# PARC-projects/video-query-algorithms

Measured on AMD Instinct MI355X. Metric: clips/sec TSN feature-extract, higher is better.
Workload: dtype f32; 1 GPU; configs[1]: TSN BN-Inception RGB, 224x224x3, T=3, B=32/GPU (96 crops/step), crops in HBM; global_batch=32, parallelism=dp1

## Files before the change

video-query-algorithms_amd/csrc/vq_tsn.hip:

```cpp
#include <algorithm>
#include <cmath>
#include <cstring>
#include <map>
#include <set>
#include <tuple>
#include <type_traits>
#include <vector>

#include "vq_common.h"
#include "vq_tsn_kernels.h"
#include "host/vq_block_pool.h"

using namespace vq;

typedef float floatx16 __attribute__((ext_vector_type(16)));
typedef float floatx4 __attribute__((ext_vector_type(4)));
typedef unsigned uintx4 __attribute__((__vector_size__(4 * sizeof(unsigned))));

__global__ void preprocess_kernel(const uint8_t* __restrict__ src, float* __restrict__ dst, int64_t nchunk, int C, int Cpad,
                                  const float* __restrict__ mean) {
    const int64_t i = (int64_t)blockIdx.x * blockDim.x + threadIdx.x;
    if (i >= nchunk) return;
    const int cpp = Cpad >> 2;
    const int64_t p = i / cpp;
// ... 294 lines not shown
    floatx16 acc[TM][TN];
#pragma unroll
    for (int i = 0; i < TM; ++i)
#pragma unroll
        for (int j = 0; j < TN; ++j)
#pragma unroll
            for (int r = 0; r < 16; ++r) acc[i][j][r] = 0.f;

    floatx4 bias_v[TN];
    ConvSeg seg_v[TN];
#pragma unroll
    for (int j = 0; j < TN; ++j) {
        const int nb_ = n0 + wn * (BN / WN) + 32 * j;
        const int n = nb_ + (lane & 7) * 4;
        bias_v[j] = *reinterpret_cast<const floatx4*>(a.bias + (n < a.Cout ? n : 0));
        seg_v[j] = a.segs[ks * a.seg_stride + (nb_ < a.Cout ? nb_ >> 5 : 0)];
    }

    const int nk = (a.ksplit > 1 ? a.k_per : a.Kp) / BK;
    VQ_LOAD_TILES(0)
    VQ_STORE_TILES(0)
    __syncthreads();
    for (int kc = 0; kc < nk; ++kc) {
        const int buf = kc & 1;
        if (kc + 1 < nk) VQ_LOAD_TILES(kc + 1)
#pragma unroll
        for (int kk = 0; kk < BK / 8; ++kk) {
            floatx4 af[TM], bf[TN];
#pragma unroll
            for (int i = 0; i < TM; ++i) af[i] = *reinterpret_cast<const floatx4*>(&sm.a[buf][arow0 + 32 * i][kk * 8 + half * 4]);
#pragma unroll
            for (int j = 0; j < TN; ++j) bf[j] = *reinterpret_cast<const floatx4*>(&sm.b[buf][brow0 + 32 * j][kk * 8 + half * 4]);
#pragma unroll
            for (int s = 0; s < 4; ++s)
#pragma unroll
                for (int i = 0; i < TM; ++i)
#pragma unroll
                    for (int j = 0; j < TN; ++j)
                        acc[i][j] = __builtin_amdgcn_mfma_f32_32x32x2f32(af[i][s], bf[j][s], acc[i][j], 0, 0, 0);
        }
        if (kc + 1 < nk) VQ_STORE_TILES(buf ^ 1)
        __syncthreads();
    }

    VQ_EPILOGUE()
#undef VQ_LOAD_TILES
#undef VQ_STORE_TILES
}

#ifndef VQ_PIPE_WPE
#define VQ_PIPE_WPE 4
#endif
template <int BM, int BN, int WM, int WN, int BK, bool SMALL_CIN>
__global__ __launch_bounds__(256) __attribute__((amdgpu_waves_per_eu(BM * BN == 128 * 64 && BK == 16 ? VQ_PIPE_WPE : 1, 8)))
void conv_igemm_pipe_kernel(ConvArgs a) {
    static_assert(WM * WN == 4, "4 waves per workgroup");
    constexpr int NT = 256;
    constexpr int TM = BM / WM / 32, TN = BN / WN / 32;
    constexpr int CPR = BK / 4;
    constexpr int NA = (BM * CPR + NT - 1) / NT, NB = (BN * CPR + NT - 1) / NT;
    constexpr int NKK = BK / 8;
    constexpr int MFK = 4 * TM * TN;
    constexpr int NMF = NKK * MFK;
    constexpr int NFR = TM + TN;
    constexpr int NG = NA + NB;
    constexpr int NFREE = NMF - (NKK - 1) * NFR;
    static_assert(NFREE >= 2 * NG, "not enough MFMA gaps for the staging slices");
    constexpr bool EARLY = (NKK - 1) * (MFK - NFR) >= NG && NFREE - NFR >= 2 * NG;
    extern __shared__ __attribute__((aligned(16))) char smem_raw[];
    ConvSmem<BM, BN, BK>& sm = *reinterpret_cast<ConvSmem<BM, BN, BK>*>(smem_raw);

    const int tid = threadIdx.x;
    const int n_tiles = a.tiles_m * a.tiles_n;
    const int ks = a.ksplit > 1 ? (int)blockIdx.x / n_tiles : 0;
    const int kbeg = ks * a.k_per;
    const int tile = xcd_remap(blockIdx.x - ks * n_tiles, n_tiles);
    const int tm = (int)magic_div((unsigned)tile, a.m_tiles_n);
    const int m0 = tm * BM;
    const int n0 = (tile - tm * a.tiles_n) * BN;
    const unsigned img0 = full_div((unsigned)m0, a.d_howo), rem0 = (unsigned)m0 - img0 * (unsigned)(a.Ho * a.Wo);
    const unsigned oh0 = full_div(rem0, a.d_wo), ow0 = rem0 - oh0 * (unsigned)a.Wo;

    const __amdgpu_buffer_rsrc_t in_rsrc = __builtin_amdgcn_make_buffer_rsrc(const_cast<float*>(a.in), 0, a.in_bytes, 0x00020000);
    const __amdgpu_buffer_rsrc_t w_rsrc = __builtin_amdgcn_make_buffer_rsrc(const_cast<float*>(a.w), 0, a.w_bytes, 0x00020000);
    int a_off[NA];
    unsigned long long a_mask[NA];
    int a_row[NA], a_col[NA];
    const unsigned HW = (unsigned)(a.H * a.W);
#pragma unroll
    for (int i = 0; i < NA; ++i) {
        const int c = tid + NT * i;
        a_row[i] = c / CPR;
        a_col[i] = c % CPR;
        const bool ok = m0 + a_row[i] < a.M && a_row[i] < BM;
        const unsigned lin = ow0 + (unsigned)a_row[i];
        const unsigned q1 = umul24(lin, a.s_wo) >> kRecipShift;
        const unsigned ly = oh0 + q1;
        const unsigned q2 = umul24(ly, a.s_ho) >> kRecipShift;
        const int ow = (int)(lin - umul24(q1, (unsigned)a.Wo)), oh = (int)(ly - umul24(q2, (unsigned)a.Ho));
        const int ih0 = imul24(oh, a.stride) - a.pad, iw0 = imul24(ow, a.stride) - a.pad;
        a_off[i] = (imul24((int)umul24(img0 + q2, HW) + imul24(ih0, a.W) + iw0, a.Cs_in) + a.coff_in + (SMALL_CIN ? 0 : imul24(a_col[i], a.col_off))) * 4;
        unsigned long long mask = 0;
        for (int th = 0; th < a.k; ++th)
            for (int tw = 0; tw < a.kw; ++tw)
                if (ok && (unsigned)(ih0 + th) < (unsigned)a.H && (unsigned)(iw0 + tw) < (unsigned)a.W) mask |= 1ull << (th * a.kw + tw);
        a_mask[i] = mask;
    }
    unsigned b_off[NB];
    int b_row[NB], b_col[NB];
#pragma unroll
    for (int i = 0; i < NB; ++i) {
        const int c = tid + NT * i;
        b_row[i] = c / CPR;
        b_col[i] = c % CPR;
        const int n = n0 + b_row[i];
        b_off[i] = (n < a.Cout && b_row[i] < BN) ? (unsigned)((imul24(n, a.Kp) + b_col[i] * 4 + kbeg) * 4) : 0xFFFFFFFFu;
    }

    floatx4 ra[2][NA], rb[2][NB];
    int kh = 0, kw = 0, c0 = 0, tap = 0;
    unsigned a_voff[NA];
    if (!SMALL_CIN && kbeg > 0) {
        tap = kbeg / a.Cin;
        c0 = kbeg - tap * a.Cin;
        kh = tap / a.kw;
        kw = tap - kh * a.kw;
    }
    {
        const int tap_pix0 = ((kh * a.W + kw) * a.Cs_in) * 4;
#pragma unroll
        for (int i = 0; i < NA; ++i) a_voff[i] = ((a_mask[i] >> tap) & 1ull) ? (unsigned)(a_off[i] + tap_pix0) : 0xFFFFFFFFu;
    }
    const int c_step = a.c_step ? a.c_step : BK;
    const unsigned cpt = (unsigned)a.Cin >> 2, inv_cpt = 65536u / cpt + 1u, inv_k = 65536u / (unsigned)a.kw + 1u;

    const int wave = __builtin_amdgcn_readfirstlane(tid >> 6), lane = tid & 63, l31 = lane & 31, half = lane >> 5;
    const int wm = wave / WN, wn = wave % WN;
    const int arow0 = wm * (BM / WM) + l31, brow0 = wn * (BN / WN) + l31;
    floatx16 acc[TM][TN];
#pragma unroll
    for (int i = 0; i < TM; ++i)
#pragma unroll
        for (int j = 0; j < TN; ++j)
#pragma unroll
            for (int r = 0; r < 16; ++r) acc[i][j][r] = 0.f;
    floatx4 bias_v[TN];
    ConvSeg seg_v[TN];
#pragma unroll
    for (int j = 0; j < TN; ++j) {
        const int nb_ = n0 + wn * (BN / WN) + 32 * j;
        const int n = nb_ + (lane & 7) * 4;
        bias_v[j] = *reinterpret_cast<const floatx4*>(a.bias + (n < a.Cout ? n : 0));
        seg_v[j] = a.segs[ks * a.seg_stride + (nb_ < a.Cout ? nb_ >> 5 : 0)];
    }

#define VQ_G_LOAD(IDX, KC, SET)                                                                                \
    {                                                                                                          \
        if ((IDX) < NA) {                                                                                      \
            const int ii = (IDX) < NA ? (IDX) : 0;                                                             \
            unsigned off;                                                                                      \
            if (SMALL_CIN) {                                                                                   \
                const unsigned g_ = (unsigned)(KC) * CPR + a_col[ii];                                          \
                const unsigned tap_ = (g_ * inv_cpt) >> 16, c4_ = g_ - tap_ * cpt;                             \
                const unsigned th_ = (tap_ * inv_k) >> 16, tw_ = tap_ - th_ * a.kw;                            \
                const unsigned ok_ = (unsigned)(a_mask[ii] >> (tap_ & 63u)) & (tap_ < 64u ? 1u : 0u);          \
                off = ok_ ? (unsigned)(a_off[ii] + (int)(((th_ * a.W + tw_) * a.Cs_in + c4_ * 4) * 4)) : 0xFFFFFFFFu; \
            } else {                                                                                           \
                off = a_voff[ii];                                                                              \
            }                                                                                                  \
            ra[SET][ii] = __builtin_bit_cast(floatx4, __builtin_amdgcn_raw_buffer_load_b128(in_rsrc, off, SMALL_CIN ? 0 : c0 * 4, 0)); \
        } else {                                                                                               \
            const int ii = (IDX) >= NA ? (IDX) - NA : 0;                                                       \
            rb[SET][ii] = __builtin_bit_cast(floatx4, __builtin_amdgcn_raw_buffer_load_b128(w_rsrc, b_off[ii], (KC) * (BK * 4), 0)); \
        }                                                                                                      \
    }
#define VQ_G_STORE(IDX, BUF, SET)                                                                              \
    {                                                                                                          \
        if ((IDX) < NA) {                                                                                      \
            const int ii = (IDX) < NA ? (IDX) : 0;                                                             \
            if ((BM * CPR) % NT == 0 || a_row[ii] < BM)                                                        \
                *reinterpret_cast<floatx4*>(&sm.a[BUF][a_row[ii]][a_col[ii] * 4]) = ra[SET][ii];               \
        } else {                                                                                               \
            const int ii = (IDX) >= NA ? (IDX) - NA : 0;                                                       \
            if ((BN * CPR) % NT == 0 || b_row[ii] < BN)                                                        \
                *reinterpret_cast<floatx4*>(&sm.b[BUF][b_row[ii]][b_col[ii] * 4]) = rb[SET][ii];               \
        }                                                                                                      \
    }
#define VQ_ADVANCE_TAP()                                                                     \
    if (!SMALL_CIN) {                                                                        \
        c0 += c_step;                                                                        \
        if (c0 >= a.Cin) {                                                                   \
            c0 = 0;                                                                          \
            ++tap;                                                                           \
            if (++kw == a.kw) {                                                              \
                kw = 0;                                                                      \
                ++kh;                                                                        \
            }                                                                                \
            asm volatile("" ::: "memory");                  \
            const int tap_pix = ((kh * a.W + kw) * a.Cs_in) * 4;                             \
            _Pragma("unroll") for (int i = 0; i < NA; ++i)                                   \
                a_voff[i] = ((a_mask[i] >> tap) & 1ull) ? (unsigned)(a_off[i] + tap_pix) : 0xFFFFFFFFu; \
        }                                                                                    \
    }
#define VQ_PIPE_STEP(BUF, KC, DO_STORE, DO_LOAD, SS, SL)                                                       \
    {                                                                                                          \
        if (!EARLY) {                                                                                          \
            _Pragma("unroll") for (int i = 0; i < TM; ++i)                                                     \
                fa[0][i] = *reinterpret_cast<const floatx4*>(&sm.a[BUF][arow0 + 32 * i][half * 4]);            \
            _Pragma("unroll") for (int j = 0; j < TN; ++j)                                                     \
                fb[0][j] = *reinterpret_cast<const floatx4*>(&sm.b[BUF][brow0 + 32 * j][half * 4]);            \
        }                                                                                                      \
        _Pragma("unroll") for (int q = 0; q < NMF; ++q) {                                                      \
            const int kk = q / MFK, r = q % MFK, s_ = r / (TM * TN), i_ = (r / TN) % TM, j_ = r % TN;          \
            acc[i_][j_] = __builtin_amdgcn_mfma_f32_32x32x2f32(fa[kk & 1][i_][s_], fb[kk & 1][j_][s_], acc[i_][j_], 0, 0, 0); \
            if (kk + 1 < NKK && r < NFR) {                                                                     \
                if (r < TM)                                                                                    \
                    fa[(kk + 1) & 1][r < TM ? r : 0] = *reinterpret_cast<const floatx4*>(                      \
                        &sm.a[BUF][arow0 + 32 * (r < TM ? r : 0)][(kk + 1) * 8 + half * 4]);                   \
                else                                                                                           \
                    fb[(kk + 1) & 1][r >= TM ? r - TM : 0] = *reinterpret_cast<const floatx4*>(                \
                        &sm.b[BUF][brow0 + 32 * (r >= TM ? r - TM : 0)][(kk + 1) * 8 + half * 4]);             \
            } else if (EARLY && (DO_STORE) && kk + 1 == NKK && r < NFR) {                                      \
                if (r < TM)                                                                                    \
                    fa[0][r < TM ? r : 0] = *reinterpret_cast<const floatx4*>(                                 \
                        &sm.a[(BUF) ^ 1][arow0 + 32 * (r < TM ? r : 0)][half * 4]);                            \
                else                                                                                           \
                    fb[0][r >= TM ? r - TM : 0] = *reinterpret_cast<const floatx4*>(                           \
                        &sm.b[(BUF) ^ 1][brow0 + 32 * (r >= TM ? r - TM : 0)][half * 4]);                      \
            } else {                                                                                           \
                const int fidx = q - (kk + 1 < NKK ? (kk + 1) * NFR : (NKK - 1) * NFR + (EARLY && (DO_STORE) ? NFR : 0)); \
                if ((DO_STORE) && fidx < NG) {                                                                 \
                    VQ_G_STORE(fidx < NG ? fidx : 0, (BUF) ^ 1, SS)                                            \
                    if (EARLY && fidx == NG - 1) __syncthreads();            \
                } else if ((DO_LOAD) && fidx >= NG && fidx < 2 * NG)                                           \
                    VQ_G_LOAD(fidx - NG < NG ? fidx - NG : 0, (KC) + 2, SL)                                    \
            }                                                                                                  \
            __builtin_amdgcn_sched_barrier(0);                                                                 \
        }                                                                                                      \
    }

    const int nk = (a.ksplit > 1 ? a.k_per : a.Kp) / BK;
    _Pragma("unroll") for (int i = 0; i < NG; ++i) VQ_G_LOAD(i, 0, 0)
    _Pragma("unroll") for (int i = 0; i < NG; ++i) VQ_G_STORE(i, 0, 0)
    if (nk > 1) {
        VQ_ADVANCE_TAP()
        _Pragma("unroll") for (int i = 0; i < NG; ++i) VQ_G_LOAD(i, 1, 1)
    }
    __syncthreads();
    floatx4 fa[2][TM], fb[2][TN];
    if (EARLY) {
#pragma unroll
        for (int i = 0; i < TM; ++i) fa[0][i] = *reinterpret_cast<const floatx4*>(&sm.a[0][arow0 + 32 * i][half * 4]);
#pragma unroll
        for (int j = 0; j < TN; ++j) fb[0][j] = *reinterpret_cast<const floatx4*>(&sm.b[0][brow0 + 32 * j][half * 4]);
    }
#define VQ_END_BARRIER()                                                     \
    {                                                                        \
        if (EARLY) {                                                         \
            asm volatile("s_waitcnt lgkmcnt(%0)" ::"n"(NFR) : "memory");     \
            __builtin_amdgcn_s_barrier();                                    \
            asm volatile("" ::: "memory");                                   \
        } else {                                                             \
            __syncthreads();                                                 \
        }                                                                    \
    }
    const int n_steady = nk > 2 ? nk - 2 : 0;
    int kc = 0;
    for (; kc + 1 < n_steady; kc += 2) {
        VQ_ADVANCE_TAP()
        VQ_PIPE_STEP(0, kc, true, true, 1, 0)
        VQ_END_BARRIER()
        VQ_ADVANCE_TAP()
        VQ_PIPE_STEP(1, kc + 1, true, true, 0, 1)
        VQ_END_BARRIER()
    }
    if (kc < n_steady) {
        VQ_ADVANCE_TAP()
        VQ_PIPE_STEP(0, kc, true, true, 1, 0)
        VQ_END_BARRIER()
        ++kc;
    }
    if (kc + 1 < nk) {
        if (kc & 1) {
            VQ_PIPE_STEP(1, kc, true, false, 0, 0)
        } else {
            VQ_PIPE_STEP(0, kc, true, false, 1, 1)
        }
        VQ_END_BARRIER()
        ++kc;
    }
    if (kc & 1) {
        VQ_PIPE_STEP(1, kc, false, false, 0, 0)
    } else {
        VQ_PIPE_STEP(0, kc, false, false, 0, 0)
    }
    VQ_EPILOGUE_BUF()
#undef VQ_G_LOAD
#undef VQ_G_STORE
#undef VQ_ADVANCE_TAP
#undef VQ_PIPE_STEP
#undef VQ_END_BARRIER
}

template <int BM, int BN, int WM, int WN>
__global__ __launch_bounds__(256) void pool_gemm_kernel(ConvArgs a) {
    static_assert(WM * WN == 4, "4 waves per workgroup");
    static_assert(BM == 64 || BM == 128, "two staged chunks per thread and slab");
    constexpr int TM = BM / WM / 32, TN = BN / WN / 32;
    constexpr int SLAB = 2048 / BM;
    constexpr int CPS = SLAB / 4;
    constexpr int GS = SLAB / 8;
    extern __shared__ __attribute__((aligned(16))) char smem_raw[];
    float* As = reinterpret_cast<float*>(smem_raw);
    const int K = a.Cin, pitch = K + 4;
    const int tid = threadIdx.x;
    const int tile = xcd_remap(blockIdx.x, a.tiles_m * a.tiles_n);
    const int m0 = (tile / a.tiles_n) * BM, n0 = (tile % a.tiles_n) * BN;
    const __amdgpu_buffer_rsrc_t in_rsrc = __builtin_amdgcn_make_buffer_rsrc(const_cast<float*>(a.in), 0, a.in_bytes, 0x00020000);
    const __amdgpu_buffer_rsrc_t w_rsrc = __builtin_amdgcn_make_buffer_rsrc(const_cast<float*>(a.w), 0, a.w_bytes, 0x00020000);

    const int wave = tid >> 6, lane = tid & 63, l31 = lane & 31, half = lane >> 5;
    const int wm = wave / WN, wn = wave % WN;
    floatx4 bias_v[TN];
    ConvSeg seg_v[TN];
    unsigned b_voff[TN];
#pragma unroll
    for (int j = 0; j < TN; ++j) {
        const int nb_ = n0 + wn * (BN / WN) + 32 * j;
        const int n = nb_ + (lane & 7) * 4;
        bias_v[j] = *reinterpret_cast<const floatx4*>(a.bias + (n < a.Cout ? n : 0));
        seg_v[j] = a.segs[nb_ < a.Cout ? nb_ >> 5 : 0];
        b_voff[j] = nb_ + l31 < a.Cout ? (unsigned)(((nb_ + l31) * a.Kp + half * 4) * 4) : 0xFFFFFFFFu;
    }

    unsigned tap_base[2], tap_ok[2];
    int a_dst[2];
    const int px = a.Cs_in * 4, rowb = a.W * px;
    {
        const int HoWo = a.Ho * a.Wo;
#pragma unroll
        for (int u = 0; u < 2; ++u) {
            const int idx = tid + 256 * u, row = idx / CPS, col = idx % CPS;
            const int m = m0 + row;
            const bool ok = m < a.M;
            const int mm = ok ? m : 0;
            const int n_img = mm / HoWo, rem = mm - n_img * HoWo;
            const int oh = rem / a.Wo, ow = rem - oh * a.Wo;
            const int ih0 = oh * a.pool_s, iw0 = ow * a.pool_s;
            tap_base[u] = ok ? (unsigned)((((n_img * a.H + ih0) * a.W + iw0) * a.Cs_in + a.coff_in + col * 4) * 4) : 0xFFFFFFFFu;
            const int nvy = min(3, a.H - ih0), nvx = min(3, a.W - iw0);
            unsigned mask = 0;
#pragma unroll
            for (int t = 0; t < 9; ++t)
                if (ok && t / 3 < nvy && t % 3 < nvx) mask |= 1u << t;
            tap_ok[u] = mask;
            a_dst[u] = row * pitch + col * 4;
        }
    }
    floatx4 v[2][9];
#define VQ_PG_TAPS(S)                                                                                               \
    _Pragma("unroll") for (int u = 0; u < 2; ++u) {                                                                 \
        unsigned inside = tap_ok[u];                                                                                \
        asm volatile("" : "+v"(inside));  \
        _Pragma("unroll") for (int t = 0; t < 9; ++t)                                                               \
            v[u][t] = __builtin_bit_cast(floatx4, __builtin_amdgcn_raw_buffer_load_b128(                            \
                in_rsrc, tap_base[u] + (((inside >> t) & 1u) ? (unsigned)((t / 3) * rowb + (t % 3) * px) : 0u), (S) * (SLAB * 4), 0)); \
    }
#define VQ_PG_POOL(S)                                                                                               \
    _Pragma("unroll") for (int u = 0; u < 2; ++u) {                                                                 \
        floatx4 r;                                                                                                  \
        _Pragma("unroll") for (int e = 0; e < 4; ++e) {                                                             \
            const float x = __builtin_fmaxf(__builtin_fmaxf(v[u][0][e], v[u][1][e]), v[u][2][e]);                  \
            const float y = __builtin_fmaxf(__builtin_fmaxf(v[u][3][e], v[u][4][e]), v[u][5][e]);                  \
            const float z = __builtin_fmaxf(__builtin_fmaxf(v[u][6][e], v[u][7][e]), v[u][8][e]);                  \
            r[e] = __builtin_fmaxf(__builtin_fmaxf(x, y), z);                                                       \
        }                                                                                                           \
        *reinterpret_cast<floatx4*>(As + a_dst[u] + (S) * SLAB) = r;                                                \
    }

    floatx16 acc[TM][TN];
#pragma unroll
    for (int i = 0; i < TM; ++i)
#pragma unroll
        for (int j = 0; j < TN; ++j)
#pragma unroll
            for (int r = 0; r < 16; ++r) acc[i][j][r] = 0.f;
    const float* a_frag = As + (wm * (BM / WM) + l31) * pitch + half * 4;
    floatx4 fa[2][TM], fbs[2][GS][TN];
#define VQ_PG_FETCH_B(SET, S)                                                                                       \
    _Pragma("unroll") for (int q = 0; q < GS; ++q)                                                                  \
        _Pragma("unroll") for (int j = 0; j < TN; ++j)                                                              \
            fbs[SET][q][j] = __builtin_bit_cast(floatx4, __builtin_amdgcn_raw_buffer_load_b128(w_rsrc, b_voff[j], ((S) * GS + q) * 32, 0));
#define VQ_PG_FETCH_A(SET, G)                                                                                       \
    _Pragma("unroll") for (int i = 0; i < TM; ++i)                                                                  \
        fa[SET][i] = *reinterpret_cast<const floatx4*>(a_frag + 32 * i * pitch + (G) * 8);
#define VQ_PG_MFMA(SET, BSET, Q)                                                                                    \
    _Pragma("unroll") for (int s_ = 0; s_ < 4; ++s_)                                                                \
        _Pragma("unroll") for (int i = 0; i < TM; ++i)                                                              \
            _Pragma("unroll") for (int j = 0; j < TN; ++j)                                                          \
                acc[i][j] = __builtin_amdgcn_mfma_f32_32x32x2f32(fa[SET][i][s_], fbs[BSET][Q][j][s_], acc[i][j], 0, 0, 0);
#define VQ_PG_SLAB(S, BSET)                                                                                         \
    {                                                                                                               \
        const bool more = (S) + 1 < ns;                                                                             \
        if (more) {                                                                                                 \
            VQ_PG_FETCH_B((BSET) ^ 1, (S) + 1)                                                                      \
            VQ_PG_TAPS((S) + 1)                                              \
        }                                                                                                           \
        VQ_PG_FETCH_A(0, (S) * GS)                                                                                  \
        __builtin_amdgcn_sched_barrier(0);                                                                          \
        _Pragma("unroll") for (int q = 0; q < GS; ++q) {                                                            \
            if (q + 1 < GS) VQ_PG_FETCH_A((q + 1) & 1, (S) * GS + q + 1)                                            \
            __builtin_amdgcn_sched_barrier(0);                                                                      \
            VQ_PG_MFMA(q & 1, BSET, q)                                                                              \
            __builtin_amdgcn_sched_barrier(0);                                                                      \
        }                                                                                                           \
        if (more) {                                                                                                 \
            VQ_PG_POOL((S) + 1)                                                                                     \
            __syncthreads();                                  \
        }                                                                                                           \
    }

    const int ns = K / SLAB;
    VQ_PG_FETCH_B(0, 0)
    VQ_PG_TAPS(0)
    VQ_PG_POOL(0)
    __syncthreads();
    int s = 0;
    for (; s + 1 < ns; s += 2) {
        VQ_PG_SLAB(s, 0)
        VQ_PG_SLAB(s + 1, 1)
    }
    if (s < ns) VQ_PG_SLAB(s, 0)
#undef VQ_PG_SLAB
#undef VQ_PG_TAPS
#undef VQ_PG_POOL
#undef VQ_PG_FETCH_A
#undef VQ_PG_FETCH_B
#undef VQ_PG_MFMA
    VQ_EPILOGUE()
}

template <bool IS_MAX>
__global__ __launch_bounds__(256) void pool_kernel(PoolArgs a) {
    const int64_t i = (int64_t)blockIdx.x * blockDim.x + threadIdx.x;
    if (i < a.total) pool_one<IS_MAX>(a, i);
}

__global__ void gavgpool_kernel(const float* __restrict__ in, float* __restrict__ out, int n, int HW, int Cs_in, int coff_in,
                                int C, int Cs_out, int coff_out) {
    const int i = blockIdx.x * blockDim.x + threadIdx.x;
    if (i >= n * C) return;
    const int c = i % C, img = i / C;
    const float* p = in + (size_t)img * HW * Cs_in + coff_in + c;
    float acc = 0.f;
    for (int q = 0; q < HW; ++q) acc += p[(size_t)q * Cs_in];
    out[(size_t)img * Cs_out + coff_out + c] = acc / (float)HW;
}

__global__ void splitk_combine_kernel(const float* __restrict__ part, int ksplit, size_t slice_stride, int M, int Cout,
                                      const float* __restrict__ bias, int relu, float* __restrict__ out, int Cs_out) {
    const int64_t i = (int64_t)blockIdx.x * blockDim.x + threadIdx.x;
    const int c4 = Cout / 4;
    if (i >= (int64_t)M * c4) return;
    const int m = (int)(i / c4), n = (int)(i - (int64_t)m * c4) * 4;
    floatx4 v = *reinterpret_cast<const floatx4*>(part + (size_t)m * Cout + n);
    for (int q = 1; q < ksplit; ++q) v += *reinterpret_cast<const floatx4*>(part + q * slice_stride + (size_t)m * Cout + n);
    v += *reinterpret_cast<const floatx4*>(bias + n);
    if (relu) {
        v[0] = fmaxf(v[0], 0.f);
        v[1] = fmaxf(v[1], 0.f);
        v[2] = fmaxf(v[2], 0.f);
        v[3] = fmaxf(v[3], 0.f);
    }
    *reinterpret_cast<floatx4*>(out + (size_t)m * Cs_out + n) = v;
}

constexpr int kMaxFusedT = 16;
__global__ void gavgpool_consensus_kernel(const float* __restrict__ in, float* __restrict__ out, double* __restrict__ feat, int T,
                                          int HW, int Cs_in, int coff_in, int C, int Cs_out, int coff_out) {
    __shared__ float pooled[kMaxFusedT][64];
    const int c = blockIdx.x * 64 + threadIdx.x, t = threadIdx.y, b = blockIdx.y;
    float v = 0.f;
    if (c < C) {
        const int img = b * T + t;
        const float* p = in + (size_t)img * HW * Cs_in + coff_in + c;
        float acc = 0.f;
        int q = 0;
        for (; q + 7 <= HW; q += 7) {
            float x[7];
#pragma unroll
            for (int u = 0; u < 7; ++u) x[u] = p[(size_t)(q + u) * Cs_in];
#pragma unroll
            for (int u = 0; u < 7; ++u) acc += x[u];
        }
        for (; q < HW; ++q) acc += p[(size_t)q * Cs_in];
        v = acc / (float)HW;
        out[(size_t)img * Cs_out + coff_out + c] = v;
    }
    pooled[t][threadIdx.x] = v;
    __syncthreads();
    if (t == 0 && c < C) {
        double cons = (double)pooled[0][threadIdx.x];
        for (int s = 1; s < T; ++s) cons = cons + (double)pooled[s][threadIdx.x];
        feat[(size_t)b * C + c] = cons / (double)T;
    }
}

__global__ void consensus_kernel(const float* __restrict__ per_snippet, double* __restrict__ feat, int B, int T, int D, int Cs) {
    const int i = blockIdx.x * blockDim.x + threadIdx.x;
    if (i >= B * D) return;
    const int d = i % D, b = i / D;
    double acc = (double)per_snippet[(size_t)(b * T) * Cs + d];
    for (int t = 1; t < T; ++t) acc = acc + (double)per_snippet[(size_t)(b * T + t) * Cs + d];
    feat[i] = acc / (double)T;
}

static inline double first_layer_k2c(const vq_input_desc& in, const vq_layer_desc& L) {
    if (L.src != 0) return (double)L.k * L.k * L.cin;
    const int k = (in.s2d_pad >= 0 && in.s2d_kernel > 0) ? in.s2d_kernel : L.k;
    return (double)k * k * in.c;
}

static inline bool is_wino(int op) { return op == VQ_OP_CONV_WINOGRAD || op == VQ_OP_CONV_WINOGRAD16; }
static inline bool is_conv(int op) { return op == VQ_OP_CONV || is_wino(op); }

struct LaunchItem {
    int kind = 0;
    std::vector<int> layers;
    int max_crops = 0;
};

struct vq_tsn {
    std::mutex mu;
    int device = 0;
    hipStream_t stream = nullptr;
    int cus = 256;
    int max_crops = 0;
    int in_channels = 0;
    vq_input_desc input = {0, 0, 0, -1, 0};
    std::vector<vq_tensor_desc> tensors;
    std::vector<vq_layer_desc> layers;
    std::vector<LaunchItem> items;
    std::vector<int> item_of_layer;
    int consensus_layer = -1;
    std::map<int, std::vector<int>> tuned;
    std::map<int, int> split_pref;
    std::set<int> tuned_borrowed;
    bool autotune = true;
    bool group_wino = true;
    bool group_pool = true;
    bool poison = false;
    int forced_tile = -1;
    std::vector<float*> slots;
    std::vector<size_t> slot_bytes;
    size_t blob_bytes = 0;
    float* zeros = nullptr;
    ConvSeg* seg_table = nullptr;
    std::vector<int> seg_table_off;
    std::vector<int> ksplit;
    float* split_scratch = nullptr;
    size_t split_slice_floats = 0;
    size_t split_crop_floats = 0;
    float* zero_bias = nullptr;
    float* blob = nullptr;
    int64_t blob_floats = 0;
    int feature_slot = -1, D = 0;
    uint8_t* crops_dev = nullptr;
    size_t crops_cap = 0;
    float* mean_dev = nullptr;
    std::vector<float> mean_cached;
    double* feat_dev = nullptr;
    double flops_per_crop = 0;
    int last_crops = 0;
    int cur_T = 1;
    bool fused_consensus = false;
    int profile_depth = 0;
    int profile_count = 0;
    int profile_every = 1;
    int profile_tick = 0;
    bool profile_split = false;
    std::vector<hipEvent_t> events;
    int crop_off = 0;
    int n_split = 1;
    std::vector<int> split_parts;
    hipStream_t ls = nullptr;
    hipEvent_t ev_start = nullptr, ev_stop = nullptr;
    std::vector<hipStream_t> split_streams;
    hipEvent_t fork_ev = nullptr;
    std::vector<hipEvent_t> join_ev;
};

static vq::BlockPool& device_pool() {
    static vq::BlockPool p(vq::BlockPool::cap_from_env());
    return p;
}
void vq::device_pool_trim() {
    for (void* blk : device_pool().drain()) (void)hipFree(blk);
}
static hipError_t pool_alloc(int device, size_t bytes, void** out) {
    if (void* blk = device_pool().take(device, bytes)) {
        *out = blk;
        return hipSuccess;
    }
    hipError_t e = hipMalloc(out, bytes);
    if (e == hipErrorOutOfMemory) {
        (void)hipGetLastError();
        vq::device_pool_trim();
        e = hipMalloc(out, bytes);
    }
    return e;
}
static void pool_free(int device, void* p, size_t bytes) {
    if (!p) return;
    if (!device_pool().give(device, p, bytes)) (void)hipFree(p);
}

static void tsn_free(vq_tsn* net) {
    for (hipEvent_t e : net->events) (void)hipEventDestroy(e);
    net->events.clear();
    for (hipEvent_t e : net->join_ev)
        if (e) (void)hipEventDestroy(e);
    if (net->fork_ev) (void)hipEventDestroy(net->fork_ev);
    for (hipStream_t st : net->split_streams)
        if (st) (void)hipStreamDestroy(st);
    for (size_t i = 0; i < net->slots.size(); ++i) pool_free(net->device, net->slots[i], i < net->slot_bytes.size() ? net->slot_bytes[i] : 0);
    pool_free(net->device, net->blob, net->blob_bytes);
    if (net->zeros) (void)hipFree(net->zeros);
    if (net->seg_table) (void)hipFree(net->seg_table);
    pool_free(net->device, net->split_scratch, net->split_slice_floats * 4 * sizeof(float));
    if (net->zero_bias) (void)hipFree(net->zero_bias);
    if (net->crops_dev) (void)hipFree(net->crops_dev);
    if (net->mean_dev) (void)hipFree(net->mean_dev);
    if (net->feat_dev) (void)hipFree(net->feat_dev);
}

enum : int { kConv = 1, kPipe = 2, kPool = 4, kGemm = 8 };

constexpr size_t kPoolGemmMaxLds = 64 * 1024;
static size_t pool_gemm_lds(int bm, int K) { return std::max((size_t)bm * (K + 4) * sizeof(float), (size_t)4 * 32 * 36 * sizeof(float)); }

static bool pixel_walk_ok(const ConvArgs& a) {
    const long long n_img = cdiv(a.M, a.Ho * a.Wo);
    return n_img * a.H * a.W < (1 << 23) && a.Cs_in < (1 << 23) && a.Kp < (1 << 23) && a.Cout < (1 << 23) && a.stride < (1 << 23) &&
           recip22_ok((unsigned)a.Wo, (unsigned)a.Wo + 128u) && recip22_ok((unsigned)a.Ho, (unsigned)a.Ho + 130u);
}

template <int BM, int BN, int WM, int WN, int BK, int KERNEL, bool SMALL>
static int launch_conv_t(vq_tsn* net, ConvArgs& a) {
    a.tiles_m = cdiv(a.M, BM);
    a.tiles_n = cdiv(a.Cout, BN);
    void (*kern)(ConvArgs);
    size_t lds = sizeof(ConvSmem<BM, BN, BK>), lds_max = lds;
    if constexpr (KERNEL == kPipe) {
        VQ_REQUIRE(pixel_walk_ok(a) && (unsigned long long)a.tiles_m * a.tiles_n * a.tiles_n < 0x100000000ull,
                   "pipelined convolution: shape outside the range of its reciprocal divisions");
        a.m_tiles_n = a.tiles_n == 1 ? 0u : (unsigned)(0x100000000ull / (unsigned)a.tiles_n) + 1u;
        a.d_howo = full_div_for((unsigned)(a.Ho * a.Wo));
        a.d_wo = full_div_for((unsigned)a.Wo);
        a.s_wo = recip22((unsigned)a.Wo);
        a.s_ho = recip22((unsigned)a.Ho);
        kern = conv_igemm_pipe_kernel<BM, BN, WM, WN, BK, SMALL>;
    } else if constexpr (KERNEL == kGemm) {
        VQ_REQUIRE(a.pool_k == 3 && a.Cin % 32 == 0 && a.Kp == a.Cin, "pool_gemm_kernel: a 3x3 window over a multiple of 32 channels");
        kern = pool_gemm_kernel<BM, BN, WM, WN>;
        lds = pool_gemm_lds(BM, a.Cin);
        lds_max = kPoolGemmMaxLds;
    } else {
        kern = conv_igemm_kernel<BM, BN, WM, WN, BK, SMALL, KERNEL == kPool>;
    }
    VQ_DYN_LDS(kern, lds_max);
    VQ_LAUNCH(kern, a.tiles_m * a.tiles_n * a.ksplit, 256, lds, net->ls, net->ev_start, net->ev_stop, a);
    VQ_CHECK_LAUNCH();
    return VQ_OK;
}

typedef int (*ConvLaunch)(vq_tsn*, ConvArgs&);

struct ConvTile {
    int bm, bn, bk;
    int pipe;
    ConvLaunch conv[2];
    ConvLaunch piped[2];
    ConvLaunch pooled;
};

template <int BM, int BN, int BK, int WM, int WN, int HAS>
constexpr ConvTile tiling() {
    ConvTile t{BM, BN, BK, (HAS & kGemm) ? 3 : (HAS & kPipe) ? 1 : 0, {}, {}, nullptr};
    if constexpr ((HAS & (kConv | kPipe)) != 0) {
        t.conv[0] = launch_conv_t<BM, BN, WM, WN, BK, kConv, false>;
        t.conv[1] = launch_conv_t<BM, BN, WM, WN, BK, kConv, true>;
    }
    if constexpr ((HAS & kPipe) != 0) {
        t.piped[0] = launch_conv_t<BM, BN, WM, WN, BK, kPipe, false>;
        t.piped[1] = launch_conv_t<BM, BN, WM, WN, BK, kPipe, true>;
    }
    if constexpr ((HAS & kPool) != 0) t.pooled = launch_conv_t<BM, BN, WM, WN, BK, kPool, false>;
    if constexpr ((HAS & kGemm) != 0) t.pooled = launch_conv_t<BM, BN, WM, WN, BK, kGemm, false>;
    return t;
}

static constexpr ConvTile kTiles[] = {
    tiling<128, 128, 32, 2, 2, kConv>(), tiling<128, 128, 16, 2, 2, kConv | kPool>(),
    tiling<128, 96, 32, 4, 1, kConv>(),  tiling<128, 96, 16, 4, 1, kConv | kPool>(),
    tiling<128, 64, 32, 2, 2, kConv>(),  tiling<128, 64, 16, 2, 2, kConv | kPool>(),
    tiling<64, 128, 32, 2, 2, kConv | kPool>(), tiling<64, 128, 16, 2, 2, kConv | kPool>(),
    tiling<64, 64, 32, 2, 2, kConv | kPool>(),  tiling<64, 64, 16, 2, 2, kConv | kPool>(),
    tiling<128, 32, 32, 4, 1, kConv>(),  tiling<128, 32, 16, 4, 1, kConv | kPool>(),
    tiling<32, 128, 32, 1, 4, kConv>(),  tiling<32, 128, 16, 1, 4, kConv>(),
    tiling<128, 128, 32, 2, 2, kPipe>(), tiling<128, 128, 16, 2, 2, kPipe>(),
    tiling<128, 96, 32, 4, 1, kPipe>(),  tiling<128, 96, 16, 4, 1, kPipe>(),
    tiling<128, 64, 32, 2, 2, kPipe>(),  tiling<128, 64, 16, 2, 2, kPipe>(),
    tiling<64, 128, 32, 2, 2, kPipe>(),  tiling<64, 128, 16, 2, 2, kPipe>(),
    tiling<64, 64, 32, 2, 2, kPipe>(),   tiling<64, 64, 16, 2, 2, kPipe>(),
    tiling<128, 32, 32, 4, 1, kPipe>(),  tiling<128, 32, 16, 4, 1, kPipe>(),
    tiling<32, 128, 32, 1, 4, kPipe>(),  tiling<32, 128, 16, 1, 4, kPipe>(),
    tiling<64, 256, 16, 1, 4, kPool>(), tiling<64, 256, 8, 1, 4, kGemm>(), tiling<64, 64, 8, 2, 2, kGemm>(), tiling<128, 64, 8, 2, 2, kGemm>()};
constexpr int kNumTiles = (int)(sizeof(kTiles) / sizeof(kTiles[0]));

static int tile_index(int bm, int bn, int bk, int pipe) {
    for (int i = 0; i < kNumTiles; ++i)
        if (kTiles[i].bm == bm && kTiles[i].bn == bn && kTiles[i].bk == bk && kTiles[i].pipe == pipe) return i;
    return -1;
}

static bool pooled_ok(const ConvTile& t, int K) { return t.pooled && (t.pipe != 3 || pool_gemm_lds(t.bm, K) <= kPoolGemmMaxLds); }

static bool tile_candidate(const vq_layer_desc& L, const ConvTile& t, bool timed) {
    if (!timed) return t.pipe == 0 && t.bk == 32 && t.conv[0];
    if (L.pre_pool_k > 0 ? !pooled_ok(t, L.cin) : !t.conv[0]) return false;
    return t.bn < 2 * ((L.cout + 63) / 64 * 64);
}

static int heuristic_tile(const vq_tsn* net, int li, int n_crops) {
    const vq_layer_desc& L = net->layers[li];
    const vq_tensor_desc& td = net->tensors[L.dst];
    const int M = n_crops * td.h * td.w, N = L.cout;
    int best = 0;
    double bs = -1;
    for (int i = 0; i < kNumTiles; ++i) {
        const ConvTile& t = kTiles[i];
        if (!tile_candidate(L, t, false)) continue;
        const long long tiles = (long long)cdiv(M, t.bm) * cdiv(N, t.bn);
        const double per_cu = (double)tiles / net->cus;
        const double balance = per_cu / std::ceil(per_cu);
        const double padding = ((double)M * N) / ((double)tiles * t.bm * t.bn);
        const double area = (double)t.bm * t.bn;
        const double intrinsic = area >= 128 * 128 ? 1.0 : area >= 128 * 96 ? 0.97 : area >= 128 * 64 ? 0.92 : area >= 64 * 64 ? 0.8 : 0.7;
        const double sc = balance * padding * intrinsic;
        if (sc > bs) {
            bs = sc;
            best = i;
        }
    }
    return best;
}

static ConvLaunch conv_launch(const vq_tsn* net, int li, const ConvArgs& a, bool stem_rows, int ti) {
    const ConvTile* t = &kTiles[ti];
    if (net->layers[li].pre_pool_k > 0) {
        if (!pooled_ok(*t, a.Cin)) ti = tile_index(std::min(t->bm, 128), std::min(t->bn, 128), 16, 0);
        return ti < 0 ? nullptr : kTiles[ti].pooled;
    }
    if (stem_rows) ti = tile_index(t->bm, t->bn, 16, t->pipe);
    if (ti < 0) return nullptr;
    t = &kTiles[ti];
    const bool small = (a.Cin % t->bk) != 0;
    return t->piped[small] && pixel_walk_ok(a) ? t->piped[small] : t->conv[small];
}

static void fill_conv_args(vq_tsn* net, int li, int n_crops, ConvArgs& a) {
    const vq_layer_desc& L = net->layers[li];
    const vq_tensor_desc& ts = net->tensors[L.src];
    const vq_tensor_desc& td = net->tensors[L.dst];
    a.in = net->slots[L.src] + (size_t)net->crop_off * ts.h * ts.w * ts.c;
    a.out = net->slots[L.dst];
    a.out_row0 = net->crop_off * td.h * td.w;
    a.w = net->blob + L.w_off;
    a.bias = net->blob + L.b_off;
    a.zeros = net->zeros;
    a.segs = net->seg_table + net->seg_table_off[li];
    a.H = ts.h;
    a.W = ts.w;
    a.Cs_in = ts.c;
    a.coff_in = L.src_coff;
    a.Cin = L.cin;
    a.Ho = td.h;
    a.Wo = td.w;
    a.Cs_out = td.c;
    a.coff_out = L.dst_coff;
    a.Cout = L.cout;
    a.k = L.k;
    a.kw = L.k;
    a.col_off = 4;
    a.c_step = 0;
    a.stride = L.stride;
    a.pad = L.pad;
    a.M = n_crops * td.h * td.w;
    a.Kp = (L.k * L.k * L.cin + KPAD - 1) / KPAD * KPAD;
    a.relu = L.relu;
    a.pool_k = L.pre_pool_k;
    a.pool_s = L.pre_pool_stride;
    a.ksplit = 1;
    a.k_per = 0;
    a.seg_stride = 0;
    a.tiles_m = a.tiles_n = 0;
    a.in_bytes = (unsigned)((size_t)n_crops * ts.h * ts.w * ts.c * sizeof(float));
    a.w_bytes = (unsigned)((size_t)L.cout * a.Kp * sizeof(float));
}

static int launch_conv_layer(vq_tsn* net, int li, int n_crops, int tile_idx) {
    ConvArgs a;
    fill_conv_args(net, li, n_crops, a);
    const vq_layer_desc& L = net->layers[li];
    const bool stem_rows = L.src == 0 && net->input.s2d_pad >= 0 && net->input.s2d_order == 1;
    if (stem_rows) {
        a.k = a.kw = 1;
        a.Cin = 4 * L.k * L.cin;
        a.col_off = net->tensors[L.src].w * net->tensors[L.src].c;
        a.c_step = 4;
        a.Kp = stem_rows_kp(net->input.c);
        a.w_bytes = (unsigned)((size_t)L.cout * a.Kp * sizeof(float));
    } else if (L.pad == 0 && L.k > 1 && L.cin == net->tensors[L.src].c && L.src_coff == 0) {
        a.kw = 1;
        a.Cin = L.k * L.cin;
    }
    const ConvLaunch run = conv_launch(net, li, a, stem_rows, tile_idx);
    const ConvTile& t = kTiles[tile_idx];
    if (!run) return fail(VQ_E_INVALID, "layer %d: no kernel for tile %dx%dx%d pipe=%d", li, t.bm, t.bn, t.bk, t.pipe);
    if (net->ksplit[li] == 1) return run(net, a);
    const hipEvent_t e0 = net->ev_start, e1 = net->ev_stop;
    a.ksplit = net->ksplit[li];
    a.k_per = a.Kp / a.ksplit;
    a.seg_stride = (L.cout + 31) / 32;
    a.bias = net->zero_bias;
    a.out_row0 = (int)cdiv((int64_t)net->crop_off * (int64_t)net->split_crop_floats, (int64_t)L.cout);
    net->ev_stop = nullptr;
    int rc = run(net, a);
    net->ev_stop = e1;
    if (rc != VQ_OK) return rc;
    net->ev_start = nullptr;
    const vq_tensor_desc& td = net->tensors[L.dst];
    float* out = net->slots[L.dst] + (size_t)net->crop_off * td.h * td.w * td.c + L.dst_coff;
    const int64_t work = (int64_t)a.M * (L.cout / 4);
    VQ_LAUNCH(splitk_combine_kernel, (unsigned)cdiv(work, 256), 256, 0, net->ls, net->ev_start, net->ev_stop,
              net->split_scratch + (size_t)a.out_row0 * L.cout, a.ksplit, net->split_slice_floats, a.M, L.cout, net->blob + L.b_off, L.relu, out, td.c);
    net->ev_start = e0;
    VQ_CHECK_LAUNCH();
    return VQ_OK;
}

static void fill_wino_job(vq_tsn* net, int li, int n_crops, WinoJob& a, int variant) {
    const vq_layer_desc& L = net->layers[li];
    const vq_tensor_desc& ts = net->tensors[L.src];
    const vq_tensor_desc& td = net->tensors[L.dst];
    memset(&a, 0, sizeof a);
    a.in = net->slots[L.src] + (size_t)net->crop_off * ts.h * ts.w * ts.c;
    a.u = net->blob + L.w_off;
    a.bias = net->blob + L.b_off;
    a.out = net->slots[L.dst] + (size_t)net->crop_off * td.h * td.w * td.c;
    a.H = ts.h;
    a.W = ts.w;
    a.Cs_in = ts.c;
    a.coff_in = L.src_coff;
    a.Cin = L.cin;
    a.Cs_out = td.c;
    a.coff_out = L.dst_coff;
    a.Cout = L.cout;
    a.th = (ts.h + 1) / 2;
    a.tw = (ts.w + 1) / 2;
    a.P = n_crops * a.th * a.tw;
    a.relu = L.relu;
    a.t16 = L.op == VQ_OP_CONV_WINOGRAD16 && variant >= 2;
    if (a.t16) a.u += (size_t)16 * L.cout * L.cin;
    a.in_bytes = (unsigned)((size_t)n_crops * ts.h * ts.w * ts.c * sizeof(float));
    a.out_bytes = (unsigned)((size_t)n_crops * td.h * td.w * td.c * sizeof(float));
    a.u_bytes = (unsigned)((size_t)16 * L.cout * L.cin * sizeof(float));
}

static void fill_pool_args(vq_tsn* net, int li, int n_crops, PoolArgs& a) {
    const vq_layer_desc& L = net->layers[li];
    const vq_tensor_desc& ts = net->tensors[L.src];
    const vq_tensor_desc& td = net->tensors[L.dst];
    memset(&a, 0, sizeof a);
    a.in = net->slots[L.src] + (size_t)net->crop_off * ts.h * ts.w * ts.c;
    a.out = net->slots[L.dst] + (size_t)net->crop_off * td.h * td.w * td.c;
    a.H = ts.h;
    a.W = ts.w;
    a.Cs_in = ts.c;
    a.coff_in = L.src_coff;
    a.C = L.cin;
    a.Ho = td.h;
    a.Wo = td.w;
    a.Cs_out = td.c;
    a.coff_out = L.dst_coff;
    a.k = L.k;
    a.stride = L.stride;
    a.pad = L.pad;
    a.is_max = L.op == VQ_OP_MAXPOOL;
    a.total = (int64_t)n_crops * td.h * td.w * (L.cin / 4);
    a.bias = (L.op == VQ_OP_AVGPOOL && L.has_bias) ? net->blob + L.b_off : nullptr;
    a.relu = (L.op == VQ_OP_AVGPOOL) ? L.relu : 0;
}

static int launch_wino_layers(vq_tsn* net, const std::vector<int>& members, int n_crops, int variant) {
    WinoGroup g;
    memset(&g, 0, sizeof g);
    for (int li : members) {
        if (is_wino(net->layers[li].op)) {
            VQ_REQUIRE(g.n_jobs < kWinoMaxJobs, "a Winograd launch carries at most %d convolutions", kWinoMaxJobs);
            fill_wino_job(net, li, n_crops, g.job[g.n_jobs++], variant);
        } else {
            VQ_REQUIRE(g.n_pools < kWinoMaxPools, "a Winograd launch carries at most %d pooling layers", kWinoMaxPools);
            fill_pool_args(net, li, n_crops, g.pool[g.n_pools++]);
        }
    }
    bool both = true;
    for (int li : members)
        if (net->layers[li].op == VQ_OP_CONV_WINOGRAD) both = false;
    if (variant >= 2 && !both) {
        variant -= 2;
        for (int q = 0; q < g.n_jobs; ++q) VQ_REQUIRE(!g.job[q].t16, "internal: mixed Winograd layouts in one launch");
    }
    return launch_wino_group(g, variant, net->ls, net->ev_start, net->ev_stop);
}

static int run_layer(vq_tsn* net, int li, int n_crops, int tune_key);

static int run_item(vq_tsn* net, const LaunchItem& it, int crop0, int n_crops, int tune_key) {
    const hipEvent_t e0 = net->ev_start, e1 = net->ev_stop;
    for (int done = 0; done < n_crops;) {
        const int n = std::min(n_crops - done, it.max_crops);
        net->crop_off = crop0 + done;
        net->ev_start = done == 0 ? e0 : nullptr;
        net->ev_stop = done + n == n_crops ? e1 : nullptr;
        int rc;
        if (it.kind == 1) {
            auto tn = net->tuned.find(tune_key);
            rc = launch_wino_layers(net, it.layers, n, tn != net->tuned.end() ? tn->second[it.layers[0]] : 0);
        } else {
            rc = run_layer(net, it.layers[0], n, tune_key);
        }
        if (rc != VQ_OK) {
            net->crop_off = 0;
            net->ev_start = net->ev_stop = nullptr;
            return rc;
        }
        done += n;
    }
    net->crop_off = 0;
    net->ev_start = net->ev_stop = nullptr;
    return VQ_OK;
}

constexpr int kPairedKey = 1 << 24;
static inline int tile_key(int n_crops, bool paired) { return n_crops + (paired ? kPairedKey : 0); }

struct EventSet {
    std::vector<hipEvent_t> ev;
    ~EventSet() {
        for (hipEvent_t e : ev)
            if (e) (void)hipEventDestroy(e);
    }
};

static int autotune(vq_tsn* net, int n_crops, bool paired) {
    const int key = tile_key(n_crops, paired);
    std::vector<int>& choice = net->tuned[key];
    choice.assign(net->layers.size(), 0);
    net->tuned_borrowed.erase(key);
    net->ls = net->stream;
    const int ways = paired ? std::max(1, std::min(net->n_split, net->max_crops / n_crops)) : 1;
    EventSet events;
// ... 930 lines not shown
```

Baseline: 12840 clips/s.

## Share overlapping pool window taps between paired output pixels in pool-GEMM kernel

Each thread now handles two horizontally adjacent pooled pixels and, when both sit in the same image row, loads the shared middle column once, cutting tap loads from 18 to 15 per slab. Window rows are folded into running maxima and, for larger tiles, interleaved with the MFMA k-groups. B-fragment prefetch moves from a double buffer to a per-group single buffer, and bias/segment loads move to the epilogue, both to reduce register pressure. An occupancy hint (waves_per_eu) and a smaller LDS cap aim for more resident waves, at the cost of more complex scheduling and a non-paired fallback variant.

```diff
diff --git a/video-query-algorithms_amd/csrc/vq_tsn.hip b/video-query-algorithms_amd/csrc/vq_tsn.hip
--- a/video-query-algorithms_amd/csrc/vq_tsn.hip
+++ b/video-query-algorithms_amd/csrc/vq_tsn.hip
@@ -620,14 +620,16 @@
 #undef VQ_END_BARRIER
 }
 
-template <int BM, int BN, int WM, int WN>
-__global__ __launch_bounds__(256) void pool_gemm_kernel(ConvArgs a) {
+template <int BM, int BN, int WM, int WN, bool PAIRED>
+__global__ __launch_bounds__(256) __attribute__((amdgpu_waves_per_eu(PAIRED ? 3 : 1, 8))) void pool_gemm_kernel(ConvArgs a) {
     static_assert(WM * WN == 4, "4 waves per workgroup");
     static_assert(BM == 64 || BM == 128, "two staged chunks per thread and slab");
     constexpr int TM = BM / WM / 32, TN = BN / WN / 32;
     constexpr int SLAB = 2048 / BM;
     constexpr int CPS = SLAB / 4;
     constexpr int GS = SLAB / 8;
+    constexpr bool BY_ROW = TM * TN >= 4;
+    static_assert(!BY_ROW || GS >= 3, "a window row per k-group");
     extern __shared__ __attribute__((aligned(16))) char smem_raw[];
     float* As = reinterpret_cast<float*>(smem_raw);
     const int K = a.Cin, pitch = K + 4;
@@ -639,27 +641,24 @@
 
     const int wave = tid >> 6, lane = tid & 63, l31 = lane & 31, half = lane >> 5;
     const int wm = wave / WN, wn = wave % WN;
-    floatx4 bias_v[TN];
-    ConvSeg seg_v[TN];
     unsigned b_voff[TN];
 #pragma unroll
     for (int j = 0; j < TN; ++j) {
         const int nb_ = n0 + wn * (BN / WN) + 32 * j;
-        const int n = nb_ + (lane & 7) * 4;
-        bias_v[j] = *reinterpret_cast<const floatx4*>(a.bias + (n < a.Cout ? n : 0));
-        seg_v[j] = a.segs[nb_ < a.Cout ? nb_ >> 5 : 0];
         b_voff[j] = nb_ + l31 < a.Cout ? (unsigned)(((nb_ + l31) * a.Kp + half * 4) * 4) : 0xFFFFFFFFu;
     }
 
-    unsigned tap_base[2], tap_ok[2];
-    int a_dst[2];
+    unsigned tap_base[2], tap_ok;
+    int a_dst;
     const int px = a.Cs_in * 4, rowb = a.W * px;
     {
         const int HoWo = a.Ho * a.Wo;
+        const int row = (tid / CPS) * 2, col = tid % CPS;
+        int img[2], ohs[2];
+        tap_ok = 0;
 #pragma unroll
         for (int u = 0; u < 2; ++u) {
-            const int idx = tid + 256 * u, row = idx / CPS, col = idx % CPS;
-            const int m = m0 + row;
+            const int m = m0 + row + u;
             const bool ok = m < a.M;
             const int mm = ok ? m : 0;
             const int n_img = mm / HoWo, rem = mm - n_img * HoWo;
@@ -667,95 +666,140 @@
             const int ih0 = oh * a.pool_s, iw0 = ow * a.pool_s;
             tap_base[u] = ok ? (unsigned)((((n_img * a.H + ih0) * a.W + iw0) * a.Cs_in + a.coff_in + col * 4) * 4) : 0xFFFFFFFFu;
             const int nvy = min(3, a.H - ih0), nvx = min(3, a.W - iw0);
-            unsigned mask = 0;
 #pragma unroll
             for (int t = 0; t < 9; ++t)
-                if (ok && t / 3 < nvy && t % 3 < nvx) mask |= 1u << t;
-            tap_ok[u] = mask;
-            a_dst[u] = row * pitch + col * 4;
-        }
-    }
-    floatx4 v[2][9];
-#define VQ_PG_TAPS(S)                                                                                               \
-    _Pragma("unroll") for (int u = 0; u < 2; ++u) {                                                                 \
-        unsigned inside = tap_ok[u];                                                                                \
-        asm volatile("" : "+v"(inside));  \
-        _Pragma("unroll") for (int t = 0; t < 9; ++t)                                                               \
-            v[u][t] = __builtin_bit_cast(floatx4, __builtin_amdgcn_raw_buffer_load_b128(                            \
-                in_rsrc, tap_base[u] + (((inside >> t) & 1u) ? (unsigned)((t / 3) * rowb + (t % 3) * px) : 0u), (S) * (SLAB * 4), 0)); \
-    }
-#define VQ_PG_POOL(S)                                                                                               \
-    _Pragma("unroll") for (int u = 0; u < 2; ++u) {                                                                 \
-        floatx4 r;                                                                                                  \
-        _Pragma("unroll") for (int e = 0; e < 4; ++e) {                                                             \
-            const float x = __builtin_fmaxf(__builtin_fmaxf(v[u][0][e], v[u][1][e]), v[u][2][e]);                  \
-            const float y = __builtin_fmaxf(__builtin_fmaxf(v[u][3][e], v[u][4][e]), v[u][5][e]);                  \
-            const float z = __builtin_fmaxf(__builtin_fmaxf(v[u][6][e], v[u][7][e]), v[u][8][e]);                  \
-            r[e] = __builtin_fmaxf(__builtin_fmaxf(x, y), z);                                                       \
+                if (ok && t / 3 < nvy && t % 3 < nvx) tap_ok |= 1u << (9 * u + t);
+            img[u] = ok ? n_img : -1 - u;
+            ohs[u] = oh;
+        }
+        if (img[0] == img[1] && ohs[0] == ohs[1]) tap_ok |= 1u << 18;
+        a_dst = row * pitch + col * 4;
+    }
+
+    floatx4 v[3][6], pm[2];
+#define VQ_PG_TAPS(ALL, S, R)                                                                                       \
+    {                                                                                                               \
+        unsigned in = tap_ok;                                                                                       \
+        asm volatile("" : "+v"(in));  \
+        const unsigned in0 = in >> (3 * (R)), in1 = in >> (9 + 3 * (R));                                            \
+        const bool shared = (in >> 18) & 1u;                                                                        \
+        unsigned o[6];                                                                                              \
+        o[0] = tap_base[0] + ((in0 & 1u) ? (unsigned)((R) * rowb) : 0u);                                            \
+        o[1] = tap_base[0] + ((in0 & 2u) ? (unsigned)((R) * rowb + px) : 0u);                                       \
+        o[2] = tap_base[1] + ((in1 & 1u) ? (unsigned)((R) * rowb) : 0u);                                            \
+        o[3] = tap_base[1] + ((in1 & 2u) ? (unsigned)((R) * rowb + px) : 0u);                                       \
+        o[4] = tap_base[1] + ((in1 & 4u) ? (unsigned)((R) * rowb + 2 * px) : 0u);                                   \
+        if (!(ALL)) {                                                                                               \
+            o[5] = shared ? 0xFFFFFFFFu : o[2];                                                                     \
+            o[2] = shared ? o[2] : tap_base[0] + ((in0 & 4u) ? (unsigned)((R) * rowb + 2 * px) : 0u);               \
         }                                                                                                           \
-        *reinterpret_cast<floatx4*>(As + a_dst[u] + (S) * SLAB) = r;                                                \
+        _Pragma("unroll") for (int t = 0; t < ((ALL) ? 5 : 6); ++t)                                                 \
+            v[R][t] = __builtin_bit_cast(floatx4, __builtin_amdgcn_raw_buffer_load_b128(in_rsrc, o[t], (S) * (SLAB * 4), 0)); \
+    }
+#define VQ_PG_FOLD(ALL, R)                                                                                          \
+    _Pragma("unroll") for (int e = 0; e < 4; ++e) {                                                                 \
+        const float first1 = (ALL) || ((tap_ok >> 18) & 1u) ? v[R][2][e] : v[R][5][e];                              \
+        const float x0 = __builtin_fmaxf(__builtin_fmaxf(v[R][0][e], v[R][1][e]), v[R][2][e]);                      \
+        const float x1 = __builtin_fmaxf(__builtin_fmaxf(first1, v[R][3][e]), v[R][4][e]);                          \
+        pm[0][e] = (R) == 0 ? x0 : __builtin_fmaxf(pm[0][e], x0);                                                   \
+        pm[1][e] = (R) == 0 ? x1 : __builtin_fmaxf(pm[1][e], x1);                                                   \
+        asm volatile("" : "+v"(pm[0][e]), "+v"(pm[1][e]));  \
+    }
+#define VQ_PG_STORE(S)                                                                                              \
+    {                                                                                                               \
+        *reinterpret_cast<floatx4*>(As + a_dst + (S) * SLAB) = pm[0];                                               \
+        *reinterpret_cast<floatx4*>(As + a_dst + pitch + (S) * SLAB) = pm[1];                                       \
     }
 
     floatx16 acc[TM][TN];
-#pragma unroll
-    for (int i = 0; i < TM; ++i)
-#pragma unroll
-        for (int j = 0; j < TN; ++j)
-#pragma unroll
-            for (int r = 0; r < 16; ++r) acc[i][j][r] = 0.f;
     const float* a_frag = As + (wm * (BM / WM) + l31) * pitch + half * 4;
-    floatx4 fa[2][TM], fbs[2][GS][TN];
-#define VQ_PG_FETCH_B(SET, S)                                                                                       \
-    _Pragma("unroll") for (int q = 0; q < GS; ++q)                                                                  \
-        _Pragma("unroll") for (int j = 0; j < TN; ++j)                                                              \
-            fbs[SET][q][j] = __builtin_bit_cast(floatx4, __builtin_amdgcn_raw_buffer_load_b128(w_rsrc, b_voff[j], ((S) * GS + q) * 32, 0));
+    floatx4 fa[2][TM], fbs[GS][TN];
+#define VQ_PG_FETCH_B(S, Q)                                                                                         \
+    _Pragma("unroll") for (int j = 0; j < TN; ++j)                                                                  \
+        fbs[Q][j] = __builtin_bit_cast(floatx4, __builtin_amdgcn_raw_buffer_load_b128(w_rsrc, b_voff[j], ((S) * GS + (Q)) * 32, 0));
 #define VQ_PG_FETCH_A(SET, G)                                                                                       \
     _Pragma("unroll") for (int i = 0; i < TM; ++i)                                                                  \
         fa[SET][i] = *reinterpret_cast<const floatx4*>(a_frag + 32 * i * pitch + (G) * 8);
-#define VQ_PG_MFMA(SET, BSET, Q)                                                                                    \
+#define VQ_PG_MFMA(SET, Q)                                                                                          \
     _Pragma("unroll") for (int s_ = 0; s_ < 4; ++s_)                                                                \
         _Pragma("unroll") for (int i = 0; i < TM; ++i)                                                              \
             _Pragma("unroll") for (int j = 0; j < TN; ++j)                                                          \
-                acc[i][j] = __builtin_amdgcn_mfma_f32_32x32x2f32(fa[SET][i][s_], fbs[BSET][Q][j][s_], acc[i][j], 0, 0, 0);
-#define VQ_PG_SLAB(S, BSET)                                                                                         \
+                acc[i][j] = __builtin_amdgcn_mfma_f32_32x32x2f32(fa[SET][i][s_], fbs[Q][j][s_], acc[i][j], 0, 0, 0);
+#define VQ_PG_SLAB(ALL, S, MORE)                                                                                    \
     {                                                                                                               \
-        const bool more = (S) + 1 < ns;                                                                             \
-        if (more) {                                                                                                 \
-            VQ_PG_FETCH_B((BSET) ^ 1, (S) + 1)                                                                      \
-            VQ_PG_TAPS((S) + 1)                                              \
+        VQ_PG_FETCH_A(0, (S) * GS)                                                                                  \
+        if ((MORE) && !BY_ROW) {                                                                                    \
+            VQ_PG_TAPS(ALL, (S) + 1, 0)                                                                             \
+            VQ_PG_TAPS(ALL, (S) + 1, 1)                                                                             \
+            VQ_PG_TAPS(ALL, (S) + 1, 2)                                                                             \
         }                                                                                                           \
-        VQ_PG_FETCH_A(0, (S) * GS)                                                                                  \
         __builtin_amdgcn_sched_barrier(0);                                                                          \
         _Pragma("unroll") for (int q = 0; q < GS; ++q) {                                                            \
+            if ((MORE) && BY_ROW && q < 3) VQ_PG_TAPS(ALL, (S) + 1, q < 3 ? q : 0)                                  \
             if (q + 1 < GS) VQ_PG_FETCH_A((q + 1) & 1, (S) * GS + q + 1)                                            \
             __builtin_amdgcn_sched_barrier(0);                                                                      \
-            VQ_PG_MFMA(q & 1, BSET, q)                                                                              \
+            VQ_PG_MFMA(q & 1, q)                                                                                    \
+            __builtin_amdgcn_sched_barrier(0);                                                                      \
+            if (MORE) VQ_PG_FETCH_B((S) + 1, q)                                                                     \
+            if ((MORE) && BY_ROW && q < 3) VQ_PG_FOLD(ALL, q < 3 ? q : 0)                                           \
             __builtin_amdgcn_sched_barrier(0);                                                                      \
         }                                                                                                           \
-        if (more) {                                                                                                 \
-            VQ_PG_POOL((S) + 1)                                                                                     \
+        if (MORE) {                                                                                                 \
+            if (!BY_ROW) {                                                                                          \
+                VQ_PG_FOLD(ALL, 0)                                                                                  \
+                VQ_PG_FOLD(ALL, 1)                                                                                  \
+                VQ_PG_FOLD(ALL, 2)                                                                                  \
+            }                                                                                                       \
+            VQ_PG_STORE((S) + 1)                                                                                    \
             __syncthreads();                                  \
         }                                                                                                           \
     }
+#define VQ_PG_WALK(ALL)                                                                                             \
+    {                                                                                                               \
+        _Pragma("unroll") for (int q = 0; q < GS; ++q) VQ_PG_FETCH_B(0, q)                                          \
+        VQ_PG_TAPS(ALL, 0, 0)                                                                                       \
+        VQ_PG_TAPS(ALL, 0, 1)                                                                                       \
+        VQ_PG_TAPS(ALL, 0, 2)                                                                                       \
+        VQ_PG_FOLD(ALL, 0)                                                                                          \
+        VQ_PG_FOLD(ALL, 1)                                                                                          \
+        VQ_PG_FOLD(ALL, 2)                                                                                          \
+        VQ_PG_STORE(0)                                                                                              \
+        __builtin_amdgcn_sched_barrier(0);                                                                          \
+        _Pragma("unroll") for (int i = 0; i < TM; ++i)                                                              \
+            _Pragma("unroll") for (int j = 0; j < TN; ++j)                                                          \
+                _Pragma("unroll") for (int r = 0; r < 16; ++r) acc[i][j][r] = 0.f;                                  \
+        __syncthreads();                                                                                            \
+        int s = 0;                                                                                                  \
+        for (; s + 1 < ns; ++s) VQ_PG_SLAB(ALL, s, true)                                                            \
+        VQ_PG_SLAB(ALL, s, false)                                                                                   \
+    }
 
     const int ns = K / SLAB;
-    VQ_PG_FETCH_B(0, 0)
-    VQ_PG_TAPS(0)
-    VQ_PG_POOL(0)
-    __syncthreads();
-    int s = 0;
-    for (; s + 1 < ns; s += 2) {
-        VQ_PG_SLAB(s, 0)
-        VQ_PG_SLAB(s + 1, 1)
-    }
-    if (s < ns) VQ_PG_SLAB(s, 0)
+    VQ_PG_WALK(PAIRED)
+#undef VQ_PG_WALK
 #undef VQ_PG_SLAB
 #undef VQ_PG_TAPS
-#undef VQ_PG_POOL
+#undef VQ_PG_FOLD
+#undef VQ_PG_STORE
 #undef VQ_PG_FETCH_A
 #undef VQ_PG_FETCH_B
 #undef VQ_PG_MFMA
-    VQ_EPILOGUE()
+    {
+        int tid_e = tid;
+        asm volatile("" : "+v"(tid_e));
+        const int wave = tid_e >> 6, lane = tid_e & 63, l31 = lane & 31, half = lane >> 5;
+        const int wm = wave / WN, wn = wave % WN;
+        floatx4 bias_v[TN];
+        ConvSeg seg_v[TN];
+#pragma unroll
+        for (int j = 0; j < TN; ++j) {
+            const int nb_ = n0 + wn * (BN / WN) + 32 * j;
+            const int n = nb_ + (lane & 7) * 4;
+            bias_v[j] = *reinterpret_cast<const floatx4*>(a.bias + (n < a.Cout ? n : 0));
+            seg_v[j] = a.segs[nb_ < a.Cout ? nb_ >> 5 : 0];
+        }
+        VQ_EPILOGUE()
+    }
 }
 
 template <bool IS_MAX>
@@ -954,7 +998,7 @@
 
 enum : int { kConv = 1, kPipe = 2, kPool = 4, kGemm = 8 };
 
-constexpr size_t kPoolGemmMaxLds = 64 * 1024;
+constexpr size_t kPoolGemmMaxLds = 53 * 1024;
 static size_t pool_gemm_lds(int bm, int K) { return std::max((size_t)bm * (K + 4) * sizeof(float), (size_t)4 * 32 * 36 * sizeof(float)); }
 
 static bool pixel_walk_ok(const ConvArgs& a) {
@@ -980,13 +1024,19 @@
         kern = conv_igemm_pipe_kernel<BM, BN, WM, WN, BK, SMALL>;
     } else if constexpr (KERNEL == kGemm) {
         VQ_REQUIRE(a.pool_k == 3 && a.Cin % 32 == 0 && a.Kp == a.Cin, "pool_gemm_kernel: a 3x3 window over a multiple of 32 channels");
-        kern = pool_gemm_kernel<BM, BN, WM, WN>;
         lds = pool_gemm_lds(BM, a.Cin);
         lds_max = kPoolGemmMaxLds;
+        if (a.Wo % 2 == 0 && a.M % 2 == 0) {
+            kern = pool_gemm_kernel<BM, BN, WM, WN, true>;
+            VQ_DYN_LDS(kern, lds_max);
+        } else {
+            kern = pool_gemm_kernel<BM, BN, WM, WN, false>;
+            VQ_DYN_LDS(kern, lds_max);
+        }
     } else {
         kern = conv_igemm_kernel<BM, BN, WM, WN, BK, SMALL, KERNEL == kPool>;
     }
-    VQ_DYN_LDS(kern, lds_max);
+    if constexpr (KERNEL != kGemm) VQ_DYN_LDS(kern, lds_max);
     VQ_LAUNCH(kern, a.tiles_m * a.tiles_n * a.ksplit, 256, lds, net->ls, net->ev_start, net->ev_stop, a);
     VQ_CHECK_LAUNCH();
     return VQ_OK;
```

Measured after the change: 12860 clips/s, median of 6. No clear change (+0.2%).
